# anitasyang/Laplace-GNN

Measured on AMD Instinct MI355X. Metric: la.fit() samples/sec (GCN, KFAC), higher is better.
Workload: dtype f32; 1 GPU; arxiv-shaped 2-layer GCN, hessian_structure=kron (BASELINE configs[2]); num_nodes=169343, nnz=2501719, features=128, hidden=256, classes=40, n_train=90941, batch_size=10000, batches=10, parallelism=dp1 ((batch, class) units, contiguous balanced runs)

## Files before the change

### laplace-gnn_amd/csrc/paths_fused.hip

```cpp
#include "gram256.h"
#include "paths.h"

namespace lgnn {
namespace {

constexpr int kYStride = 272;
constexpr int kPlaneDwords = 512;
constexpr int kGroupDwords = 3 * kPlaneDwords;
constexpr int kYGroups = kYRows / 4;
__device__ __forceinline__ int piece_swap(int q) { return (q ^ (q >> 2)) & 1; }
__device__ __forceinline__ int piece_col(int c) { return 8 * (c >> 2) + 4 * (((c >> 1) & 1) ^ piece_swap(c >> 2)) + 2 * (c & 1); }

struct alignas(16) FusedShared {
  union {
    uint32_t pc[2][kYGroups][3][kPlaneDwords];
    float y[2][kYRows][kYStride];
  };
  int ready[4], done[4];
};
static_assert(sizeof(FusedShared) <= 160 * 1024, "the CU's LDS");

__device__ __forceinline__ int lds_min4(const int* c) {
  int4 v;
  asm volatile("ds_read_b128 %0, %1\n\ts_waitcnt lgkmcnt(0)" : "=v"(v) : "v"(uint32_t(reinterpret_cast<uintptr_t>(c))) : "memory");
  return __builtin_amdgcn_readfirstlane(min(min(v.x, v.y), min(v.z, v.w)));
}
__device__ __forceinline__ void lds_publish(int* c, int value, int lane) {
  if (lane == 0)
    asm volatile("ds_write_b32 %0, %1\n\ts_waitcnt lgkmcnt(0)" :: "v"(uint32_t(reinterpret_cast<uintptr_t>(c))), "v"(value) : "memory");
}

using i32x4 = int __attribute__((ext_vector_type(4)));
__device__ __forceinline__ i32x4 make_rsrc(const void* p, uint64_t bytes) {
  const uint64_t u = reinterpret_cast<uint64_t>(p);
  return i32x4{int(uint32_t(u)), int(uint32_t(u >> 32) & 0xffffu), int(uint32_t(bytes > 0xffffffffull ? 0xffffffffull : bytes)),
               0x00020000};
}
template <bool LIST>
struct NodeRanges {
  i32x4 prs, lrs;
  uint32_t r;
  int64_t base, cnt;
  uint32_t n0;
  __device__ __forceinline__ void init(const int32_t* __restrict__ pptr, const int32_t* __restrict__ list, int64_t n0_, int64_t N,
                                       int64_t nn, int64_t cnt_) {
    prs = make_rsrc(pptr, uint64_t(N + 1) * 4);
    lrs = make_rsrc(LIST ? list : pptr, uint64_t(LIST ? nn : 0) * 4);
    n0 = uint32_t(n0_); cnt = cnt_;
    fill(0);
  }
  __device__ __forceinline__ void fill(int64_t b) {
    base = b;
    const uint32_t ii = uint32_t(b) + (threadIdx.x & 31u);
    const bool in = int64_t(ii) < cnt;
    const uint32_t k = blockIdx.x + ii * gridDim.x;
    uint32_t node = k;
    if constexpr (LIST)
      asm volatile("buffer_load_dword %0, %1, %2, 0 offen\n\ts_waitcnt vmcnt(0)" : "=&v"(node) : "v"(in ? k * 4u : 0xfffffff0u), "s"(lrs) : "memory");
    const uint32_t off = in ? (n0 + node) * 4u + ((threadIdx.x >> 3) & 4u) : 0xfffffff0u;
    asm volatile("buffer_load_dword %0, %1, %2, 0 offen\n\ts_waitcnt vmcnt(0)" : "=&v"(r) : "v"(off), "s"(prs) : "memory");
  }
  __device__ __forceinline__ void get(int64_t i, int32_t& p0, int32_t& p1) {
    if (i - base >= 32) fill(i);
    const int l = int(i - base);
    p0 = __builtin_amdgcn_readlane(int(r), l); p1 = __builtin_amdgcn_readlane(int(r), l + 32);
  }
};

template <int OFF>
__device__ __forceinline__ void bload4(f32x4& d, uint32_t voff, const i32x4& rsrc) {
  asm volatile("buffer_load_dwordx4 %0, %1, %2, 0 offen offset:%3" : "=v"(d) : "v"(voff), "s"(rsrc), "n"(OFF) : "memory");
}
__device__ __forceinline__ void bload1(uint32_t& d, uint32_t voff, const i32x4& rsrc) {
  asm volatile("buffer_load_dword %0, %1, %2, 0 offen" : "=v"(d) : "v"(voff), "s"(rsrc) : "memory");
}
using bf16x8 = __attribute__((ext_vector_type(8))) __bf16;
using u32x4v = __attribute__((ext_vector_type(4))) uint32_t;
using u32x2v = __attribute__((ext_vector_type(2))) uint32_t;

__device__ __forceinline__ uint32_t pk_bf16(float lo, float hi) {
  using bf16x2 = __attribute__((ext_vector_type(2))) __bf16;
  const bf16x2 v = {static_cast<__bf16>(lo), static_cast<__bf16>(hi)};
  return __builtin_bit_cast(uint32_t, v);
}
__device__ __forceinline__ void split_pair(float ya, float yb, uint32_t& q0, uint32_t& q1, uint32_t& q2) {
  q0 = pk_bf16(ya, yb);
  asm("" : "+v"(q0));
  const float r1a = ya - __uint_as_float(q0 << 16), r1b = yb - __uint_as_float(q0 & 0xffff0000u);
  q1 = pk_bf16(r1a, r1b);
  asm("" : "+v"(q1));
  q2 = pk_bf16(r1a - __uint_as_float(q1 << 16), r1b - __uint_as_float(q1 & 0xffff0000u));
}

struct PTables {
  i32x4 coef, b, g, mask, pm, pv, pw;
};

struct PMeta { uint32_t oc, ob, om, w; };
__device__ __forceinline__ void meta_issue(const PTables& tb, int32_t p0, int32_t p1, int lane, PMeta& t) {
  const uint32_t q = uint32_t(max(min(p0 + lane, p1 - 1), 0)) * 4u;
  bload1(t.oc, q, tb.pm);
  bload1(t.om, q, tb.pv);
  bload1(t.w, q, tb.pw);
}
template <int YOUNGER>
__device__ __forceinline__ void meta_finish(int32_t p0, int32_t p1, int lane, uint32_t row_bytes, uint32_t mask_bytes, PMeta& t) {
  asm volatile("s_waitcnt vmcnt(%3)" : "+v"(t.oc), "+v"(t.om), "+v"(t.w) : "n"(YOUNGER) : "memory");
  const bool in = p0 + lane < p1;
  const uint32_t m = in ? t.oc : 0u, v = in ? t.om : 0u;
  t.oc = m * uint32_t(kCoefRow * 4); t.ob = m * row_bytes; t.om = v * mask_bytes;
  t.w = in ? t.w : 0u;
}

struct PLane {
  int kq;
  uint32_t oc, ob, om;
  int mshift;
};

struct POps {
  f32x4 ca[3];
  f32x4 b4, g4;
  uint32_t mw;
  float w;
};

template <bool NOBG> constexpr int kStepLoads = NOBG ? 2 : 6;
template <bool NOBG>
__device__ __forceinline__ void p_load(const PTables& tb, const PMeta& mt, int s, const PLane& pl, POps& o) {
  const int src = 4 * s + pl.kq;
  const uint32_t oc = uint32_t(__shfl(int(mt.oc), src)) + pl.oc;
  const uint32_t om = uint32_t(__shfl(int(mt.om), src)) + pl.om;
  o.w = __uint_as_float(uint32_t(__shfl(int(mt.w), src)));
  bload4<0>(o.ca[0], oc, tb.coef);
  if constexpr (!NOBG) {
    const uint32_t ob = uint32_t(__shfl(int(mt.ob), src)) + pl.ob;
    bload4<kCoefStride * 4>(o.ca[1], oc, tb.coef);
    bload4<2 * kCoefStride * 4>(o.ca[2], oc, tb.coef);
    bload4<0>(o.b4, ob, tb.b);
    bload4<0>(o.g4, ob, tb.g);
  }
  bload1(o.mw, om, tb.mask);
}
template <bool NOBG, int YOUNGER>
__device__ __forceinline__ void p_wait(POps& o) {
  if constexpr (NOBG)
    asm volatile("s_waitcnt vmcnt(%2)" : "+v"(o.ca[0]), "+v"(o.mw) : "n"(YOUNGER) : "memory");
  else
    asm volatile("s_waitcnt vmcnt(%6)" : "+v"(o.ca[0]), "+v"(o.ca[1]), "+v"(o.ca[2]), "+v"(o.b4), "+v"(o.g4), "+v"(o.mw)
                 : "n"(YOUNGER) : "memory");
}

struct PCur { float a1[3], a2[3], bb[4], gg[4]; };
struct PAlpha { u32x4v a[3], m[4]; };
constexpr uint32_t kHiHalves = 0x07060302u;
template <bool NOBG, bool HI, bool SB>
__device__ __forceinline__ void p_xform(const POps& o, const PLane& pl, PCur& c, PAlpha& al, bool bg) {
#pragma unroll
  for (int t = 0; t < 3; ++t) {
    const int tt = HI ? 3 : t;
    if (HI && t > 0) {
      if constexpr (!SB) al.a[t][0] = 0u;
      al.a[t][1] = 0u; al.a[t][2] = 0u;
      continue;
    }
    float av = o.w * o.ca[0][tt];
    asm("" : "+v"(av));
    const uint32_t h0 = __float_as_uint(av) & 0xffff0000u;
    const float r1 = av - __uint_as_float(h0);
    const float r2 = r1 - __uint_as_float(__float_as_uint(r1) & 0xffff0000u);
    if constexpr (!SB) {
      al.a[t][0] = __builtin_amdgcn_perm(__float_as_uint(r1), __float_as_uint(av), kHiHalves);
      al.a[t][1] = __float_as_uint(r2) >> 16;
    } else {
      al.a[t][1] |= h0;
      al.a[t][2] = __builtin_amdgcn_perm(__float_as_uint(r2), __float_as_uint(r1), kHiHalves);
    }
  }
  const int bits = int(o.mw >> pl.mshift);
#pragma unroll
  for (int ct = 0; ct < 4; ++ct) {
    const int on = __builtin_amdgcn_sbfe(bits, ct, 1);
    if constexpr (!SB) {
      al.m[ct][0] = uint32_t(on) & 0x3f803f80u;
      al.m[ct][1] = uint32_t(on) & 0x00003f80u;
    } else {
      al.m[ct][1] |= uint32_t(on) & 0x3f800000u;
      al.m[ct][2] = uint32_t(on) & 0x3f803f80u;
    }
  }
  if constexpr (!NOBG) {
    if (bg) {
#pragma unroll
      for (int t = 0; t < 3; ++t) {
        const int tt = HI ? 3 : t;
        c.a1[t] = (HI && t > 0) ? 0.f : o.w * o.ca[1][tt];
        c.a2[t] = (HI && t > 0) ? 0.f : o.w * o.ca[2][tt];
      }
#pragma unroll
      for (int ct = 0; ct < 4; ++ct) {
        const int on = __builtin_amdgcn_sbfe(bits, ct, 1);
        c.bb[ct] = __uint_as_float(uint32_t(on) & __float_as_uint(o.b4[ct]));
        c.gg[ct] = __uint_as_float(uint32_t(on) & __float_as_uint(o.g4[ct]));
      }
    }
  }
}
template <bool NOBG>
__device__ __forceinline__ void p_keep(const PCur& c) {
  if constexpr (!NOBG) {
    asm volatile("" :: "v"(c.a1[0]), "v"(c.a1[1]), "v"(c.a1[2]), "v"(c.a2[0]), "v"(c.a2[1]), "v"(c.a2[2]));
    asm volatile("" :: "v"(c.bb[0]), "v"(c.bb[1]), "v"(c.bb[2]), "v"(c.bb[3]), "v"(c.gg[0]), "v"(c.gg[1]), "v"(c.gg[2]), "v"(c.gg[3]));
  }
}
__device__ __forceinline__ f32x4 mfma_bf16(u32x4v a, u32x4v b, f32x4 c) {
  return __builtin_amdgcn_mfma_f32_16x16x32_bf16(__builtin_bit_cast(bf16x8, a), __builtin_bit_cast(bf16x8, b), c, 0, 0, 0);
}
__device__ __forceinline__ void p_mfma(const PCur& c, f32x4 (&y2)[3][4]) {
#pragma unroll
  for (int t = 0; t < 3; ++t)
#pragma unroll
    for (int ct = 0; ct < 4; ++ct) y2[t][ct] = __builtin_amdgcn_mfma_f32_16x16x4f32(c.a1[t], c.bb[ct], y2[t][ct], 0, 0, 0);
#pragma unroll
  for (int t = 0; t < 3; ++t)
#pragma unroll
    for (int ct = 0; ct < 4; ++ct) y2[t][ct] = __builtin_amdgcn_mfma_f32_16x16x4f32(c.a2[t], c.gg[ct], y2[t][ct], 0, 0, 0);
}
__device__ __forceinline__ void p_mfma_first(const PCur& c, f32x4 (&y2)[3][4]) {
  const f32x4 zero = {0.f, 0.f, 0.f, 0.f};
#pragma unroll
  for (int t = 0; t < 3; ++t)
#pragma unroll
    for (int ct = 0; ct < 4; ++ct) y2[t][ct] = __builtin_amdgcn_mfma_f32_16x16x4f32(c.a1[t], c.bb[ct], zero, 0, 0, 0);
#pragma unroll
  for (int t = 0; t < 3; ++t)
#pragma unroll
    for (int ct = 0; ct < 4; ++ct) y2[t][ct] = __builtin_amdgcn_mfma_f32_16x16x4f32(c.a2[t], c.gg[ct], y2[t][ct], 0, 0, 0);
}
template <bool FIRST>
__device__ __forceinline__ void p_mfma_alpha(const PAlpha& al, f32x4 (&t1)[3][4]) {
  const f32x4 zero = {0.f, 0.f, 0.f, 0.f};
#pragma unroll
  for (int t = 0; t < 3; ++t)
#pragma unroll
    for (int ct = 0; ct < 4; ++ct) t1[t][ct] = mfma_bf16(al.a[t], al.m[ct], FIRST ? zero : t1[t][ct]);
}

template <bool LIST>
struct ChunkGen {
  int64_t gi;
  int32_t gp, gend;
  int32_t pa0, pa1;
  NodeRanges<LIST> nr;
  __device__ __forceinline__ void init(const int32_t* __restrict__ pptr, const int32_t* __restrict__ list, int64_t n0, int64_t N,
                                       int64_t nn, int64_t cnt) {
    nr.init(pptr, list, n0, N, nn, cnt);
    gi = 0;
    nr.get(0, gp, gend);
    nr.get(1, pa0, pa1);
  }
  __device__ __forceinline__ void next(int64_t cnt, int32_t& q0, int32_t& q1, bool& last) {
    q0 = gp; q1 = min(gp + 64, gend);
    last = q1 >= gend;
    if (last) {
      ++gi;
      gp = pa0; gend = pa1;
      nr.get(gi + 1, pa0, pa1);
    } else {
      gp = q1;
    }
  }
};

template <bool NOBG, bool HI>
__device__ __forceinline__ void pair_body(const PTables& tb, const PMeta& mx, int sx, const PLane& pl, POps& A, POps& B, PCur& cA,
                                          PCur& cB, PAlpha& al, f32x4 (&t1)[3][4], f32x4 (&y2)[3][4], bool first, bool half) {
  constexpr int NL = kStepLoads<NOBG>;
  p_wait<NOBG, NL>(A);
  p_xform<NOBG, HI, false>(A, pl, cA, al, true);
  p_keep<NOBG>(cB);
  p_load<NOBG>(tb, mx, sx, pl, A);
  if constexpr (!NOBG) {
    if (first) p_mfma_first(cA, y2);
    else p_mfma(cA, y2);
  }
  p_wait<NOBG, NL>(B);
  p_xform<NOBG, HI, true>(B, pl, cB, al, !half);
  p_keep<NOBG>(cA);
  p_load<NOBG>(tb, mx, sx + 1, pl, B);
  if (first) p_mfma_alpha<true>(al, t1);
  else p_mfma_alpha<false>(al, t1);
  if constexpr (!NOBG)
    if (!half) p_mfma(cB, y2);
}
template <bool LIST, bool NOBG, bool HI>
__device__ __forceinline__ void product_role(const YArgs& a, const int32_t* __restrict__ pptr, const int32_t* __restrict__ list,
                                             FusedShared& sh, int64_t nn, int64_t cnt, int cg) {
  const int lane = threadIdx.x & 63;
  const int H = a.H;
  const bool path_wave = 64 * cg < H;
  if (!path_wave) return;
  PLane pl;
  const int li = lane & 15;
  pl.kq = lane >> 4;
  const int col = 64 * cg + 4 * li;
  const bool col_ok = col < H;
  pl.oc = 16u * uint32_t(li);
  pl.ob = col_ok ? 4u * uint32_t(col) : 0u;
  pl.om = col_ok ? 4u * uint32_t(col >> 5) : 0x7ffffff0u;
  pl.mshift = col & 31;
  const uint32_t row_bytes = uint32_t(H) * 4u, mask_bytes = uint32_t(a.mask_words) * 4u;
  PTables tb;
  tb.coef = make_rsrc(a.coef, uint64_t(a.n_coef) * kCoefRow * 4);
  tb.b = make_rsrc(a.bg, uint64_t(a.M) * row_bytes);
  tb.g = make_rsrc(a.bg + a.M * int64_t(H), uint64_t(a.M) * row_bytes);
  tb.mask = make_rsrc(a.mask, uint64_t(a.N) * mask_bytes);
  tb.pm = make_rsrc(a.pm, uint64_t(a.cap) * 4);
  tb.pv = make_rsrc(a.pv, uint64_t(a.cap) * 4);
  tb.pw = make_rsrc(a.pw, uint64_t(a.cap) * 4);
  const uint32_t w1_row_bytes = uint32_t(a.w1_ld) * 4u;
  const i32x4 w1rs = make_rsrc(a.W1 + int64_t(a.c0) * a.w1_ld, uint64_t(a.R - 1) * w1_row_bytes + row_bytes);
  constexpr int NL = kStepLoads<NOBG>;
  ChunkGen<LIST> gen;
  gen.init(pptr, list, a.n0, a.N, nn, cnt);
  int32_t q0c, q1c, q0n, q1n;
  bool lastc, lastn;
  gen.next(cnt, q0c, q1c, lastc);
  gen.next(cnt, q0n, q1n, lastn);
  PMeta mc, mn;
  meta_issue(tb, q0c, q1c, lane, mc);
  meta_issue(tb, q0n, q1n, lane, mn);
  meta_finish<0>(q0c, q1c, lane, row_bytes, mask_bytes, mc);
  meta_finish<0>(q0n, q1n, lane, row_bytes, mask_bytes, mn);
  POps A, B;
  p_load<NOBG>(tb, mc, 0, pl, A);
  p_load<NOBG>(tb, mc, 1, pl, B);
  f32x4 t1[3][4], y2[3][4];
#pragma unroll
  for (int t = 0; t < 3; ++t)
#pragma unroll
    for (int ct = 0; ct < 4; ++ct) { t1[t][ct] = f32x4{0.f, 0.f, 0.f, 0.f}; y2[t][ct] = f32x4{0.f, 0.f, 0.f, 0.f}; }
  PCur cA = {}, cB = {};
  PAlpha al;
#pragma unroll
  for (int t = 0; t < 3; ++t) al.a[t] = u32x4v{0u, 0u, 0u, 0u};
#pragma unroll
  for (int ct = 0; ct < 4; ++ct) al.m[ct] = u32x4v{0u, 0u, 0u, 0u};
  bool node_has = false;
  bool firstc = true;
  for (int64_t i = 0; i < cnt;) {
    int32_t q0f, q1f;
    bool lastf;
    gen.next(cnt, q0f, q1f, lastf);
    PMeta mf2;
    meta_issue(tb, q0f, q1f, lane, mf2);
    const int kch = q1c - q0c, np = max((kch + 7) >> 3, 1);
    node_has = node_has || kch > 0;
#pragma clang loop unroll(disable)
    for (int j = 0; j < np; ++j) {
      const bool more = j + 1 < np;
      PMeta mx;
      mx.oc = more ? mc.oc : mn.oc; mx.ob = more ? mc.ob : mn.ob; mx.om = more ? mc.om : mn.om; mx.w = more ? mc.w : mn.w;
      const int sx = more ? 2 * (j + 1) : 0;
      const bool first = firstc && j == 0, half = !more && 4 * (2 * j + 1) >= kch;
      pair_body<NOBG, HI>(tb, mx, sx, pl, A, B, cA, cB, al, t1, y2, first, half);
    }
    if (lastc) {
      int wl = lane;
      asm volatile("" : "+v"(wl));
      const int wkq = wl >> 4, wcol = 64 * cg + 4 * (wl & 15);
      const bool wcol_ok = wcol < H;
      const uint32_t w1_off = wcol_ok ? uint32_t(4 * wkq) * w1_row_bytes + 4u * uint32_t(wcol) : 0x7ff00000u;
      const int pc_lo = 8 * (wcol >> 2) + 4 * piece_swap(wcol >> 2), pc_hi = pc_lo ^ 4;
      f32x4 w1[3][4];
#pragma unroll
      for (int t = 0; t < 3; ++t)
#pragma unroll
        for (int r = 0; r < 4; ++r) bload4<0>(w1[t][r], w1_off + uint32_t(16 * t + r) * w1_row_bytes, w1rs);
      if (i >= 2)
        while (lds_min4(sh.done) < int(i) - 1) __builtin_amdgcn_s_sleep(2);
#pragma unroll
      for (int t = 0; t < 3; ++t)
        asm volatile("s_waitcnt vmcnt(0)" : "+v"(w1[t][0]), "+v"(w1[t][1]), "+v"(w1[t][2]), "+v"(w1[t][3]) :: "memory");
      asm volatile("s_nop 11" ::: "memory");
      __builtin_amdgcn_sched_barrier(0);
      if (node_has && wcol_ok) {
        if (a.gram_f32) {
          float (*ytile)[kYStride] = sh.y[i & 1];
#pragma unroll
          for (int t = 0; t < 3; ++t)
#pragma unroll
            for (int r = 0; r < 4; ++r) {
              f32x4 o;
#pragma unroll
              for (int ct = 0; ct < 4; ++ct) o[ct] = w1[t][r][ct] * t1[t][ct][r] + y2[t][ct][r];
              *reinterpret_cast<f32x4*>(&ytile[16 * t + 4 * wkq + r][wcol]) = o;
            }
        } else {
          uint32_t* __restrict__ grp = &sh.pc[i & 1][wkq][0][0];
#pragma unroll
          for (int t = 0; t < 3; ++t) {
            u32x4v pz[3][2];
#pragma unroll
            for (int ct = 0; ct < 4; ++ct)
#pragma unroll
              for (int rp = 0; rp < 2; ++rp) {
                const float ya = w1[t][2 * rp][ct] * t1[t][ct][2 * rp] + y2[t][ct][2 * rp];
                const float yb = w1[t][2 * rp + 1][ct] * t1[t][ct][2 * rp + 1] + y2[t][ct][2 * rp + 1];
                uint32_t q0, q1, q2;
                split_pair(ya, yb, q0, q1, q2);
                pz[0][ct >> 1][2 * (ct & 1) + rp] = q0;
                pz[1][ct >> 1][2 * (ct & 1) + rp] = q1;
                pz[2][ct >> 1][2 * (ct & 1) + rp] = q2;
              }
            uint32_t* __restrict__ g = grp + 4 * t * kGroupDwords;
            *reinterpret_cast<u32x4v*>(g + pc_lo) = pz[2][0];
            *reinterpret_cast<u32x4v*>(g + pc_hi) = pz[2][1];
            *reinterpret_cast<u32x4v*>(g + kPlaneDwords + pc_lo) = pz[0][0];
            *reinterpret_cast<u32x4v*>(g + kPlaneDwords + pc_hi) = pz[0][1];
            *reinterpret_cast<u32x4v*>(g + 2 * kPlaneDwords + pc_lo) = pz[1][0];
            *reinterpret_cast<u32x4v*>(g + 2 * kPlaneDwords + pc_hi) = pz[1][1];
          }
        }
      }
      ++i;
      lds_publish(&sh.ready[cg], int(i), lane);
#pragma unroll
      for (int t = 0; t < 3; ++t) {
        asm volatile("" : "=v"(t1[t][0]), "=v"(t1[t][1]), "=v"(t1[t][2]), "=v"(t1[t][3]));
        if constexpr (!NOBG) asm volatile("" : "=v"(y2[t][0]), "=v"(y2[t][1]), "=v"(y2[t][2]), "=v"(y2[t][3]));
      }
      node_has = false;
    }
    meta_finish<2 * NL>(q0f, q1f, lane, row_bytes, mask_bytes, mf2);
    firstc = lastc;
    q0c = q0n; q1c = q1n; lastc = lastn; mc = mn;
    q0n = q0f; q1n = q1f; lastn = lastf; mn = mf2;
  }
  asm volatile("s_waitcnt vmcnt(0)" ::: "memory");
}

template <int W>
__device__ __forceinline__ void gram16_load(const float* __restrict__ p, float (&x)[8][2]) {
#pragma unroll
  for (int b = 0; b < 8; ++b) {
    x[b][0] = tiles256_uses<W>(b) ? p[b * 32] : 0.f;
    x[b][1] = tiles256_uses<W>(b) ? p[b * 32 + 16] : 0.f;
  }
}
template <int W>
__device__ __forceinline__ void gram16_mfma(const float (&x)[8][2], f32x4 (&acc)[9][2][2]) {
#pragma unroll
  for (int s = 0; s < 9; ++s)
#pragma unroll
    for (int hi = 0; hi < 2; ++hi)
#pragma unroll
      for (int hj = 0; hj < 2; ++hj) {
        if (Tiles256<W>::si[s] == Tiles256<W>::sj[s] && hi > hj) continue;
        acc[s][hi][hj] = __builtin_amdgcn_mfma_f32_16x16x4f32(x[Tiles256<W>::si[s]][hi], x[Tiles256<W>::sj[s]][hj],
                                                              acc[s][hi][hj], 0, 0, 0);
      }
}
template <int W, bool LIST>
__device__ __forceinline__ void gram_role(const YArgs& a, const int32_t* __restrict__ pptr, const int32_t* __restrict__ list,
                                          FusedShared& sh, int64_t nn, int64_t cnt, float* __restrict__ scratch) {
  const int lane = threadIdx.x & 63;
  f32x4 acc[9][2][2];
#pragma unroll
  for (int s = 0; s < 9; ++s)
#pragma unroll
    for (int q = 0; q < 4; ++q) acc[s][q >> 1][q & 1] = f32x4{0.f, 0.f, 0.f, 0.f};
  const int nk = (a.R + 3) >> 2;
  NodeRanges<LIST> nr;
  nr.init(pptr, list, a.n0, a.N, nn, cnt);
  int32_t p0, p1;
  nr.get(0, p0, p1);
  for (int64_t i = 0; i < cnt; ++i) {
    int32_t q0, q1;
    nr.get(i + 1, q0, q1);
    while (lds_min4(sh.ready) < int(i) + 1) __builtin_amdgcn_s_sleep(2);
    if (p1 > p0) {
      const float* __restrict__ base = &sh.y[i & 1][0][0] + (lane >> 4) * kYStride + (lane & 15);
      float xa[8][2], xb[8][2];
      gram16_load<W>(base, xa);
      for (int kk = 0; kk < nk; kk += 2) {
        if (kk + 1 < nk) gram16_load<W>(base + (kk + 1) * 4 * kYStride, xb);
        __builtin_amdgcn_sched_barrier(0);
        gram16_mfma<W>(xa, acc);
        __builtin_amdgcn_sched_barrier(0);
        if (kk + 1 < nk) {
          if (kk + 2 < nk) gram16_load<W>(base + (kk + 2) * 4 * kYStride, xa);
          __builtin_amdgcn_sched_barrier(0);
          gram16_mfma<W>(xb, acc);
          __builtin_amdgcn_sched_barrier(0);
        }
      }
    }
    lds_publish(&sh.done[W], int(i) + 1, lane);
    p0 = q0; p1 = q1;
  }
  const int64_t D = a.H;
  const int li = lane & 15, lq = lane >> 4;
#pragma unroll
  for (int s = 0; s < 9; ++s)
#pragma unroll
    for (int hi = 0; hi < 2; ++hi)
#pragma unroll
      for (int hj = 0; hj < 2; ++hj) {
        if (Tiles256<W>::si[s] == Tiles256<W>::sj[s] && hi > hj) continue;
        const int64_t jj = Tiles256<W>::sj[s] * 32 + 16 * hj + li;
#pragma unroll
        for (int r = 0; r < 4; ++r) {
          const int64_t ii = Tiles256<W>::si[s] * 32 + 16 * hi + 4 * lq + r;
          if (ii < D && jj < D) atomicAdd(&scratch[ii * D + jj], acc[s][hi][hj][r]);
        }
      }
}

struct PieceBlk { u32x4v t; u32x2v y1; };

template <int W> struct GramOrder;
template <> struct GramOrder<0> { static constexpr int o[9] = {0, 3, 4, 7, 8, 1, 2, 5, 6}; };
template <> struct GramOrder<1> { static constexpr int o[9] = {7, 8, 3, 4, 5, 6, 0, 1, 2}; };
template <> struct GramOrder<2> { static constexpr int o[9] = {7, 8, 3, 4, 5, 6, 0, 1, 2}; };
template <> struct GramOrder<3> { static constexpr int o[9] = {0, 7, 3, 5, 1, 8, 4, 6, 2}; };
template <int W> __device__ __forceinline__ constexpr int gram_last_use(int b) {
  int last = -1;
  for (int p = 0; p < 9; ++p)
    if (Tiles256<W>::si[GramOrder<W>::o[p]] == b || Tiles256<W>::sj[GramOrder<W>::o[p]] == b) last = p;
  return last;
}
template <int W> __device__ __forceinline__ constexpr int gram_first_use(int b) {
  for (int p = 0; p < 9; ++p)
    if (Tiles256<W>::si[GramOrder<W>::o[p]] == b || Tiles256<W>::sj[GramOrder<W>::o[p]] == b) return p;
  return -1;
}

__device__ __forceinline__ void piece_load(const uint32_t* __restrict__ tile, int off, int b, PieceBlk (&x)[8][2]) {
  const uint32_t* __restrict__ pe = tile + off;
  const uint32_t* __restrict__ po = tile + (off ^ 4) + 32;
  const u32x2v e2 = *reinterpret_cast<const u32x2v*>(pe + b * 64), e0 = *reinterpret_cast<const u32x2v*>(pe + kPlaneDwords + b * 64);
  const u32x2v o2 = *reinterpret_cast<const u32x2v*>(po + b * 64), o0 = *reinterpret_cast<const u32x2v*>(po + kPlaneDwords + b * 64);
  x[b][0].t = u32x4v{e2[0], e2[1], e0[0], e0[1]};
  x[b][0].y1 = *reinterpret_cast<const u32x2v*>(pe + 2 * kPlaneDwords + b * 64);
  x[b][1].t = u32x4v{o2[0], o2[1], o0[0], o0[1]};
  x[b][1].y1 = *reinterpret_cast<const u32x2v*>(po + 2 * kPlaneDwords + b * 64);
}
__device__ __forceinline__ u32x4v piece_u(const PieceBlk& p) { return u32x4v{p.t[2], p.t[3], p.y1[0], p.y1[1]}; }
__device__ __forceinline__ u32x4v piece_t(const PieceBlk& p) { return p.t; }
template <int W>
__device__ __forceinline__ void piece_chunk16(PieceBlk (&x)[8][2], f32x4 (&acc)[9][2][2], const uint32_t* __restrict__ tile, int off) {
#pragma unroll
  for (int p = 0; p < 9; ++p) {
    const int s = GramOrder<W>::o[p], si = Tiles256<W>::si[s], sj = Tiles256<W>::sj[s];
#pragma unroll
    for (int b = 0; b < 8; ++b)
      if (gram_first_use<W>(b) == p)
#pragma unroll
        for (int h = 0; h < 2; ++h) asm volatile("" : "+v"(x[b][h].t), "+v"(x[b][h].y1));
    const u32x4v ua[2] = {piece_u(x[si][0]), piece_u(x[si][1])}, ta[2] = {piece_t(x[si][0]), piece_t(x[si][1])};
    const u32x4v ub[2] = {piece_u(x[sj][0]), piece_u(x[sj][1])}, tb[2] = {piece_t(x[sj][0]), piece_t(x[sj][1])};
#pragma unroll
    for (int f = 0; f < 3; ++f)
#pragma unroll
      for (int hi = 0; hi < 2; ++hi)
#pragma unroll
        for (int hj = 0; hj < 2; ++hj) {
          if (si == sj && hi > hj) continue;
          acc[s][hi][hj] = mfma_bf16(f == 1 ? ta[hi] : ua[hi], f == 2 ? tb[hj] : ub[hj], acc[s][hi][hj]);
        }
    __builtin_amdgcn_sched_barrier(0);
#pragma unroll
    for (int b = 0; b < 8; ++b)
      if (gram_last_use<W>(b) == p) piece_load(tile, off, b, x);
  }
}
template <int W>
__device__ __forceinline__ void piece_chunk8(const PieceBlk (&x)[8][2], f32x4 (&acc)[9][2][2], bool low) {
#pragma unroll
  for (int p = 0; p < 9; ++p) {
    const int s = GramOrder<W>::o[p], si = Tiles256<W>::si[s], sj = Tiles256<W>::sj[s];
    u32x4v a1[2], a2[2];
#pragma unroll
    for (int hi = 0; hi < 2; ++hi) {
      const u32x4v u = piece_u(x[si][hi]), t = piece_t(x[si][hi]);
#pragma unroll
      for (int j = 0; j < 4; ++j) { a1[hi][j] = low ? u[j] : t[j]; a2[hi][j] = low ? u[j] : 0u; }
    }
    const u32x4v ub[2] = {piece_u(x[sj][0]), piece_u(x[sj][1])}, tb[2] = {piece_t(x[sj][0]), piece_t(x[sj][1])};
#pragma unroll
    for (int f = 0; f < 2; ++f)
#pragma unroll
      for (int hi = 0; hi < 2; ++hi)
#pragma unroll
        for (int hj = 0; hj < 2; ++hj) {
          if (si == sj && hi > hj) continue;
          acc[s][hi][hj] = mfma_bf16(f == 0 ? a1[hi] : a2[hi], f == 0 ? ub[hj] : tb[hj], acc[s][hi][hj]);
        }
    __builtin_amdgcn_sched_barrier(0);
  }
}
template <int W, bool LIST>
__device__ __forceinline__ void gram_split16_role(const YArgs& a, const int32_t* __restrict__ pptr, const int32_t* __restrict__ list,
                                                  FusedShared& sh, int64_t nn, int64_t cnt, float* __restrict__ scratch) {
  const int lane = threadIdx.x & 63;
  f32x4 acc[9][2][2];
#pragma unroll
  for (int s = 0; s < 9; ++s)
#pragma unroll
    for (int q = 0; q < 4; ++q) acc[s][q >> 1][q & 1] = f32x4{0.f, 0.f, 0.f, 0.f};
  const int n8 = (a.R + 7) >> 3, n16 = n8 >> 1;
  const bool odd = n8 & 1;
  const int gq = lane >> 4;
  const int start = (n16 > 0 ? gq : gq & 1) * kGroupDwords + piece_col(lane & 15);
  const int to_odd = (4 - 2 * (gq >> 1)) * kGroupDwords;
  NodeRanges<LIST> nr;
  nr.init(pptr, list, a.n0, a.N, nn, cnt);
  int32_t p0, p1;
  nr.get(0, p0, p1);
  for (int64_t i = 0; i < cnt; ++i) {
    int32_t q0, q1;
    nr.get(i + 1, q0, q1);
    while (lds_min4(sh.ready) < int(i) + 1) __builtin_amdgcn_s_sleep(2);
    if (p1 > p0) {
      const uint32_t* __restrict__ tile = &sh.pc[i & 1][0][0][0];
      int off = start;
      PieceBlk x[8][2];
#pragma unroll
      for (int b = 0; b < 8; ++b)
        if (tiles256_uses<W>(b)) piece_load(tile, off, b, x);
      __builtin_amdgcn_sched_barrier(0);
      for (int cc = 0; cc < n16; ++cc) {
        off += cc + 1 < n16 ? 4 * kGroupDwords : odd ? to_odd : 0;
        piece_chunk16<W>(x, acc, tile, off);
      }
      if (odd) piece_chunk8<W>(x, acc, gq < 2);
    }
    lds_publish(&sh.done[W], int(i) + 1, lane);
    p0 = q0; p1 = q1;
  }
  const int64_t D = a.H;
  const int fl = int(__builtin_amdgcn_mbcnt_hi(~0u, __builtin_amdgcn_mbcnt_lo(~0u, 0u)));
  const int li = fl & 15, lq = (fl >> 4) & 3;
#pragma unroll
  for (int s = 0; s < 9; ++s)
#pragma unroll
    for (int hi = 0; hi < 2; ++hi)
#pragma unroll
      for (int hj = 0; hj < 2; ++hj) {
        if (Tiles256<W>::si[s] == Tiles256<W>::sj[s] && hi > hj) continue;
        const int64_t jj = Tiles256<W>::sj[s] * 32 + 16 * hj + li;
#pragma unroll
        for (int r = 0; r < 4; ++r) {
          const int64_t ii = Tiles256<W>::si[s] * 32 + 16 * hi + 4 * lq + r;
          if (ii < D && jj < D && (Tiles256<W>::si[s] != Tiles256<W>::sj[s] || ii <= jj)) atomicAdd(&scratch[ii * D + jj], acc[s][hi][hj][r]);
        }
      }
}

template <bool LIST>
__global__ __launch_bounds__(512, 2) void paths_fused_kernel(YArgs a, const int32_t* __restrict__ pptr,
                                                             const int32_t* __restrict__ list, float* __restrict__ scratch) {
  __shared__ FusedShared sh;
  if (int64_t(pptr[a.N]) > a.cap) return;
  for (int q = threadIdx.x; q < int(sizeof(sh.pc) / 16); q += 512) reinterpret_cast<u32x4v*>(&sh.pc[0][0][0][0])[q] = u32x4v{0u, 0u, 0u, 0u};
  if (threadIdx.x < 4) {
    sh.ready[threadIdx.x] = 64 * int(threadIdx.x) < a.H ? 0 : INT32_MAX;
    sh.done[threadIdx.x] = 0;
  }
  __syncthreads();
  const int hw = __builtin_amdgcn_readfirstlane(int(threadIdx.x >> 6));
  const int64_t stride = gridDim.x;
  const int64_t nn = LIST ? int64_t(__builtin_amdgcn_readfirstlane(*a.n_list)) : a.n1 - a.n0;
  const int64_t cnt = nn > int64_t(blockIdx.x) ? (nn - blockIdx.x + stride - 1) / stride : 0;
  switch (hw) {
    case 4: if (a.gram_f32) gram_role<0, LIST>(a, pptr, list, sh, nn, cnt, scratch); else gram_split16_role<0, LIST>(a, pptr, list, sh, nn, cnt, scratch); break;
    case 5: if (a.gram_f32) gram_role<1, LIST>(a, pptr, list, sh, nn, cnt, scratch); else gram_split16_role<1, LIST>(a, pptr, list, sh, nn, cnt, scratch); break;
    case 6: if (a.gram_f32) gram_role<2, LIST>(a, pptr, list, sh, nn, cnt, scratch); else gram_split16_role<2, LIST>(a, pptr, list, sh, nn, cnt, scratch); break;
    case 7: if (a.gram_f32) gram_role<3, LIST>(a, pptr, list, sh, nn, cnt, scratch); else gram_split16_role<3, LIST>(a, pptr, list, sh, nn, cnt, scratch); break;
    default:
      if (a.c0 != a.cb) {
        if (a.no_bg) product_role<LIST, true, true>(a, pptr, list, sh, nn, cnt, hw);
        else product_role<LIST, false, true>(a, pptr, list, sh, nn, cnt, hw);
      } else {
        if (a.no_bg) product_role<LIST, true, false>(a, pptr, list, sh, nn, cnt, hw);
        else product_role<LIST, false, false>(a, pptr, list, sh, nn, cnt, hw);
      }
      break;
  }
}

constexpr int64_t kFusedWorkgroups = 256;

}

int launch_paths_fused(lgnn_ctx* h, YArgs y, int64_t cb, int64_t ce, float* scratch, hipStream_t s) {
  LGNN_REQUIRE(y.N < (int64_t(1) << 31), "too many nodes for one launch");
  const dim3 grid{unsigned(std::min<int64_t>(y.n1 - y.n0, kFusedWorkgroups))};
  const char* e = getenv("LGNN_GRAM_F32");
  y.Y = nullptr; y.gram_f32 = e && atoi(e) != 0 ? 1 : 0;
  for (int64_t c0 = cb; c0 < ce; c0 += kYRows) {
    y.c0 = int(c0); y.R = int(std::min<int64_t>(kYRows, ce - c0));
    if (h->timing) LGNN_CALL(record_event(h, s));
    if (y.list) hipLaunchKernelGGL(paths_fused_kernel<true>, grid, dim3(512), 0, s, y, y.pptr, y.list, scratch);
    else hipLaunchKernelGGL(paths_fused_kernel<false>, grid, dim3(512), 0, s, y, y.pptr, y.list, scratch);
    LGNN_HIP_CHECK(hipGetLastError());
    if (h->timing) { LGNN_CALL(record_event(h, s)); h->ev_planes += y.R; }
  }
  return 0;
}

}
```

Before: 2.528 million samples/s.

## Stage first W1 tiles in LDS and shrink tile buffers for short row chunks

Replaces the fixed union shared-memory struct with a runtime-sized LDS layout. When the f32 gram path is used or the chunk has few rows, the first two 16-row tiles of W1 are preloaded into LDS at kernel start, so the product waves read them with ds_read instead of buffer loads in every node epilogue; only the third tile still comes from global memory. The split16 tile buffer is shortened for short chunks to make room for this. It also inserts s_nop padding before several buffer loads, adds LDS pressure and more template instantiations, and under the non-HI product path with the default split16 layout, W1 is staged only when the chunk has at most 40 rows.

```diff
diff --git a/laplace-gnn_amd/csrc/paths_fused.hip b/laplace-gnn_amd/csrc/paths_fused.hip
--- a/laplace-gnn_amd/csrc/paths_fused.hip
+++ b/laplace-gnn_amd/csrc/paths_fused.hip
@@ -11,14 +11,32 @@
 __device__ __forceinline__ int piece_swap(int q) { return (q ^ (q >> 2)) & 1; }
 __device__ __forceinline__ int piece_col(int c) { return 8 * (c >> 2) + 4 * (((c >> 1) & 1) ^ piece_swap(c >> 2)) + 2 * (c & 1); }
 
-struct alignas(16) FusedShared {
-  union {
-    uint32_t pc[2][kYGroups][3][kPlaneDwords];
-    float y[2][kYRows][kYStride];
-  };
-  int ready[4], done[4];
+constexpr int kW1Cols = 256;
+constexpr int kW1Tiles = 2;
+constexpr int kShortGroups = 10, kShortRows = 4 * kShortGroups;
+constexpr int fused_tile_dwords(bool f32, int R) {
+  return f32 ? kYRows * kYStride : kGroupDwords * (R <= kShortRows ? kShortGroups : kYGroups);
+}
+constexpr int fused_w1_tiles(bool f32, int R) { return f32 || R <= kShortRows ? kW1Tiles : 0; }
+constexpr int fused_lds_bytes(bool f32, int R) {
+  return 4 * (2 * fused_tile_dwords(f32, R) + fused_w1_tiles(f32, R) * 16 * kW1Cols) + 32;
+}
+constexpr int kFusedLdsBytes = fused_lds_bytes(false, kShortRows);
+static_assert(kFusedLdsBytes == 155680 && kFusedLdsBytes <= 160 * 1024, "the CU's LDS");
+static_assert(fused_lds_bytes(false, kYRows) <= kFusedLdsBytes && fused_lds_bytes(true, kYRows) <= kFusedLdsBytes &&
+              fused_lds_bytes(true, 1) <= kFusedLdsBytes && fused_lds_bytes(false, 1) <= kFusedLdsBytes, "every layout fits");
+struct FusedShared {
+  uint32_t* base;
+  int tile_dwords;
+  int nw;
+  __device__ __forceinline__ void init(uint32_t* lds, bool f32, int R) {
+    base = lds; tile_dwords = fused_tile_dwords(f32, R); nw = fused_w1_tiles(f32, R);
+  }
+  __device__ __forceinline__ uint32_t* tile(int64_t i) const { return base + (int(i) & 1) * tile_dwords; }
+  __device__ __forceinline__ float* w1() const { return reinterpret_cast<float*>(base + 2 * tile_dwords); }
+  __device__ __forceinline__ int* ready() const { return reinterpret_cast<int*>(base + 2 * tile_dwords + nw * 16 * kW1Cols); }
+  __device__ __forceinline__ int* done() const { return ready() + 4; }
 };
-static_assert(sizeof(FusedShared) <= 160 * 1024, "the CU's LDS");
 
 __device__ __forceinline__ int lds_min4(const int* c) {
   int4 v;
@@ -28,6 +46,17 @@
 __device__ __forceinline__ void lds_publish(int* c, int value, int lane) {
   if (lane == 0)
     asm volatile("ds_write_b32 %0, %1\n\ts_waitcnt lgkmcnt(0)" :: "v"(uint32_t(reinterpret_cast<uintptr_t>(c))), "v"(value) : "memory");
+}
+
+template <int T>
+__device__ __forceinline__ void w1_lds_read(f32x4 (&w)[4], uint32_t addr) {
+  asm volatile("ds_read_b128 %0, %1 offset:%2" : "=v"(w[0]) : "v"(addr), "n"((16 * T + 0) * kW1Cols * 4) : "memory");
+  asm volatile("ds_read_b128 %0, %1 offset:%2" : "=v"(w[1]) : "v"(addr), "n"((16 * T + 1) * kW1Cols * 4) : "memory");
+  asm volatile("ds_read_b128 %0, %1 offset:%2" : "=v"(w[2]) : "v"(addr), "n"((16 * T + 2) * kW1Cols * 4) : "memory");
+  asm volatile("ds_read_b128 %0, %1 offset:%2" : "=v"(w[3]) : "v"(addr), "n"((16 * T + 3) * kW1Cols * 4) : "memory");
+}
+__device__ __forceinline__ void w1_lds_wait(f32x4 (&w)[4]) {
+  asm volatile("s_waitcnt lgkmcnt(0)" : "+v"(w[0]), "+v"(w[1]), "+v"(w[2]), "+v"(w[3]) :: "memory");
 }
 
 using i32x4 = int __attribute__((ext_vector_type(4)));
@@ -56,9 +85,9 @@
     const uint32_t k = blockIdx.x + ii * gridDim.x;
     uint32_t node = k;
     if constexpr (LIST)
-      asm volatile("buffer_load_dword %0, %1, %2, 0 offen\n\ts_waitcnt vmcnt(0)" : "=&v"(node) : "v"(in ? k * 4u : 0xfffffff0u), "s"(lrs) : "memory");
+      asm volatile("s_nop 4\n\tbuffer_load_dword %0, %1, %2, 0 offen\n\ts_waitcnt vmcnt(0)" : "=&v"(node) : "v"(in ? k * 4u : 0xfffffff0u), "s"(lrs) : "memory");
     const uint32_t off = in ? (n0 + node) * 4u + ((threadIdx.x >> 3) & 4u) : 0xfffffff0u;
-    asm volatile("buffer_load_dword %0, %1, %2, 0 offen\n\ts_waitcnt vmcnt(0)" : "=&v"(r) : "v"(off), "s"(prs) : "memory");
+    asm volatile("s_nop 4\n\tbuffer_load_dword %0, %1, %2, 0 offen\n\ts_waitcnt vmcnt(0)" : "=&v"(r) : "v"(off), "s"(prs) : "memory");
   }
   __device__ __forceinline__ void get(int64_t i, int32_t& p0, int32_t& p1) {
     if (i - base >= 32) fill(i);
@@ -67,12 +96,17 @@
   }
 };
 
-template <int OFF>
+template <int OFF, bool PAD = false>
 __device__ __forceinline__ void bload4(f32x4& d, uint32_t voff, const i32x4& rsrc) {
-  asm volatile("buffer_load_dwordx4 %0, %1, %2, 0 offen offset:%3" : "=v"(d) : "v"(voff), "s"(rsrc), "n"(OFF) : "memory");
-}
+  if constexpr (PAD)
+    asm volatile("s_nop 4\n\tbuffer_load_dwordx4 %0, %1, %2, 0 offen offset:%3" : "=v"(d) : "v"(voff), "s"(rsrc), "n"(OFF) : "memory");
+  else
+    asm volatile("buffer_load_dwordx4 %0, %1, %2, 0 offen offset:%3" : "=v"(d) : "v"(voff), "s"(rsrc), "n"(OFF) : "memory");
+}
+template <bool PAD = false>
 __device__ __forceinline__ void bload1(uint32_t& d, uint32_t voff, const i32x4& rsrc) {
-  asm volatile("buffer_load_dword %0, %1, %2, 0 offen" : "=v"(d) : "v"(voff), "s"(rsrc) : "memory");
+  if constexpr (PAD) asm volatile("s_nop 4\n\tbuffer_load_dword %0, %1, %2, 0 offen" : "=v"(d) : "v"(voff), "s"(rsrc) : "memory");
+  else asm volatile("buffer_load_dword %0, %1, %2, 0 offen" : "=v"(d) : "v"(voff), "s"(rsrc) : "memory");
 }
 using bf16x8 = __attribute__((ext_vector_type(8))) __bf16;
 using u32x4v = __attribute__((ext_vector_type(4))) uint32_t;
@@ -99,9 +133,9 @@
 struct PMeta { uint32_t oc, ob, om, w; };
 __device__ __forceinline__ void meta_issue(const PTables& tb, int32_t p0, int32_t p1, int lane, PMeta& t) {
   const uint32_t q = uint32_t(max(min(p0 + lane, p1 - 1), 0)) * 4u;
-  bload1(t.oc, q, tb.pm);
-  bload1(t.om, q, tb.pv);
-  bload1(t.w, q, tb.pw);
+  bload1<true>(t.oc, q, tb.pm);
+  bload1<true>(t.om, q, tb.pv);
+  bload1<true>(t.w, q, tb.pw);
 }
 template <int YOUNGER>
 __device__ __forceinline__ void meta_finish(int32_t p0, int32_t p1, int lane, uint32_t row_bytes, uint32_t mask_bytes, PMeta& t) {
@@ -293,9 +327,9 @@
   if constexpr (!NOBG)
     if (!half) p_mfma(cB, y2);
 }
-template <bool LIST, bool NOBG, bool HI>
+template <bool LIST, bool NOBG, bool HI, bool W1L>
 __device__ __forceinline__ void product_role(const YArgs& a, const int32_t* __restrict__ pptr, const int32_t* __restrict__ list,
-                                             FusedShared& sh, int64_t nn, int64_t cnt, int cg) {
+                                             const FusedShared& sh, int64_t nn, int64_t cnt, int cg) {
   const int lane = threadIdx.x & 63;
   const int H = a.H;
   const bool path_wave = 64 * cg < H;
@@ -372,59 +406,80 @@
       const bool wcol_ok = wcol < H;
       const uint32_t w1_off = wcol_ok ? uint32_t(4 * wkq) * w1_row_bytes + 4u * uint32_t(wcol) : 0x7ff00000u;
       const int pc_lo = 8 * (wcol >> 2) + 4 * piece_swap(wcol >> 2), pc_hi = pc_lo ^ 4;
+      constexpr int nw = W1L ? kW1Tiles : 0;
       f32x4 w1[3][4];
 #pragma unroll
-      for (int t = 0; t < 3; ++t)
-#pragma unroll
-        for (int r = 0; r < 4; ++r) bload4<0>(w1[t][r], w1_off + uint32_t(16 * t + r) * w1_row_bytes, w1rs);
+      for (int t = nw; t < 3; ++t)
+#pragma unroll
+        for (int r = 0; r < 4; ++r) bload4<0, true>(w1[t][r], w1_off + uint32_t(16 * t + r) * w1_row_bytes, w1rs);
+      const uint32_t w1_lds = uint32_t(reinterpret_cast<uintptr_t>(sh.w1())) + uint32_t(4 * wkq * kW1Cols * 4 + 4 * wcol);
+      if constexpr (nw > 0) w1_lds_read<0>(w1[0], w1_lds);
       if (i >= 2)
-        while (lds_min4(sh.done) < int(i) - 1) __builtin_amdgcn_s_sleep(2);
-#pragma unroll
-      for (int t = 0; t < 3; ++t)
-        asm volatile("s_waitcnt vmcnt(0)" : "+v"(w1[t][0]), "+v"(w1[t][1]), "+v"(w1[t][2]), "+v"(w1[t][3]) :: "memory");
+        while (lds_min4(sh.done()) < int(i) - 1) __builtin_amdgcn_s_sleep(2);
+      if constexpr (nw > 0) w1_lds_wait(w1[0]);
+      if constexpr (nw == 0) {
+#pragma unroll
+        for (int t = 0; t < 3; ++t)
+          asm volatile("s_waitcnt vmcnt(0)" : "+v"(w1[t][0]), "+v"(w1[t][1]), "+v"(w1[t][2]), "+v"(w1[t][3]) :: "memory");
+      }
       asm volatile("s_nop 11" ::: "memory");
       __builtin_amdgcn_sched_barrier(0);
-      if (node_has && wcol_ok) {
-        if (a.gram_f32) {
-          float (*ytile)[kYStride] = sh.y[i & 1];
-#pragma unroll
-          for (int t = 0; t < 3; ++t)
-#pragma unroll
-            for (int r = 0; r < 4; ++r) {
-              f32x4 o;
-#pragma unroll
-              for (int ct = 0; ct < 4; ++ct) o[ct] = w1[t][r][ct] * t1[t][ct][r] + y2[t][ct][r];
-              *reinterpret_cast<f32x4*>(&ytile[16 * t + 4 * wkq + r][wcol]) = o;
-            }
-        } else {
-          uint32_t* __restrict__ grp = &sh.pc[i & 1][wkq][0][0];
-#pragma unroll
-          for (int t = 0; t < 3; ++t) {
-            u32x4v pz[3][2];
-#pragma unroll
-            for (int ct = 0; ct < 4; ++ct)
-#pragma unroll
-              for (int rp = 0; rp < 2; ++rp) {
-                const float ya = w1[t][2 * rp][ct] * t1[t][ct][2 * rp] + y2[t][ct][2 * rp];
-                const float yb = w1[t][2 * rp + 1][ct] * t1[t][ct][2 * rp + 1] + y2[t][ct][2 * rp + 1];
-                uint32_t q0, q1, q2;
-                split_pair(ya, yb, q0, q1, q2);
-                pz[0][ct >> 1][2 * (ct & 1) + rp] = q0;
-                pz[1][ct >> 1][2 * (ct & 1) + rp] = q1;
-                pz[2][ct >> 1][2 * (ct & 1) + rp] = q2;
-              }
-            uint32_t* __restrict__ g = grp + 4 * t * kGroupDwords;
-            *reinterpret_cast<u32x4v*>(g + pc_lo) = pz[2][0];
-            *reinterpret_cast<u32x4v*>(g + pc_hi) = pz[2][1];
-            *reinterpret_cast<u32x4v*>(g + kPlaneDwords + pc_lo) = pz[0][0];
-            *reinterpret_cast<u32x4v*>(g + kPlaneDwords + pc_hi) = pz[0][1];
-            *reinterpret_cast<u32x4v*>(g + 2 * kPlaneDwords + pc_lo) = pz[1][0];
-            *reinterpret_cast<u32x4v*>(g + 2 * kPlaneDwords + pc_hi) = pz[1][1];
+      const bool wr = node_has && wcol_ok;
+      uint32_t* __restrict__ tile = sh.tile(i);
+      auto f32_tile = [&](auto tc) __attribute__((always_inline)) {
+        constexpr int t = decltype(tc)::value;
+        if constexpr (t + 1 < nw) w1_lds_read<t + 1>(w1[t + 1], w1_lds);
+        float (*ytile)[kYStride] = reinterpret_cast<float (*)[kYStride]>(tile);
+#pragma unroll
+        for (int r = 0; r < 4; ++r) {
+          f32x4 o;
+#pragma unroll
+          for (int ct = 0; ct < 4; ++ct) o[ct] = w1[t][r][ct] * t1[t][ct][r] + y2[t][ct][r];
+          *reinterpret_cast<f32x4*>(&ytile[16 * t + 4 * wkq + r][wcol]) = o;
+        }
+        if constexpr (t + 1 < nw) w1_lds_wait(w1[t + 1]);
+      };
+      auto piece_tile = [&](auto tc) __attribute__((always_inline)) {
+        constexpr int t = decltype(tc)::value;
+        if constexpr (t + 1 < nw) w1_lds_read<t + 1>(w1[t + 1], w1_lds);
+        u32x4v pz[3][2];
+#pragma unroll
+        for (int ct = 0; ct < 4; ++ct)
+#pragma unroll
+          for (int rp = 0; rp < 2; ++rp) {
+            const float ya = w1[t][2 * rp][ct] * t1[t][ct][2 * rp] + y2[t][ct][2 * rp];
+            const float yb = w1[t][2 * rp + 1][ct] * t1[t][ct][2 * rp + 1] + y2[t][ct][2 * rp + 1];
+            uint32_t q0, q1, q2;
+            split_pair(ya, yb, q0, q1, q2);
+            pz[0][ct >> 1][2 * (ct & 1) + rp] = q0;
+            pz[1][ct >> 1][2 * (ct & 1) + rp] = q1;
+            pz[2][ct >> 1][2 * (ct & 1) + rp] = q2;
           }
+        if constexpr (t + 1 < nw) w1_lds_wait(w1[t + 1]);
+        if (t < 2 || sh.tile_dwords != kGroupDwords * kShortGroups || wkq < kShortGroups - 8) {
+          uint32_t* __restrict__ g = tile + (4 * t + wkq) * kGroupDwords;
+          *reinterpret_cast<u32x4v*>(g + pc_lo) = pz[2][0];
+          *reinterpret_cast<u32x4v*>(g + pc_hi) = pz[2][1];
+          *reinterpret_cast<u32x4v*>(g + kPlaneDwords + pc_lo) = pz[0][0];
+          *reinterpret_cast<u32x4v*>(g + kPlaneDwords + pc_hi) = pz[0][1];
+          *reinterpret_cast<u32x4v*>(g + 2 * kPlaneDwords + pc_lo) = pz[1][0];
+          *reinterpret_cast<u32x4v*>(g + 2 * kPlaneDwords + pc_hi) = pz[1][1];
         }
+      };
+      using T0 = std::integral_constant<int, 0>; using T1 = std::integral_constant<int, 1>; using T2 = std::integral_constant<int, 2>;
+      if (wr) {
+        if (a.gram_f32) { f32_tile(T0{}); f32_tile(T1{}); if constexpr (nw == 0) f32_tile(T2{}); }
+        else { piece_tile(T0{}); piece_tile(T1{}); if constexpr (nw == 0) piece_tile(T2{}); }
+      }
+      if constexpr (nw > 0) {
+        asm volatile("s_waitcnt vmcnt(0)" : "+v"(w1[2][0]), "+v"(w1[2][1]), "+v"(w1[2][2]), "+v"(w1[2][3]) :: "memory");
+        if (wr) {
+          if (a.gram_f32) f32_tile(T2{});
+          else piece_tile(T2{});
+        }
       }
       ++i;
-      lds_publish(&sh.ready[cg], int(i), lane);
+      lds_publish(sh.ready() + cg, int(i), lane);
 #pragma unroll
       for (int t = 0; t < 3; ++t) {
         asm volatile("" : "=v"(t1[t][0]), "=v"(t1[t][1]), "=v"(t1[t][2]), "=v"(t1[t][3]));
@@ -463,7 +518,7 @@
 }
 template <int W, bool LIST>
 __device__ __forceinline__ void gram_role(const YArgs& a, const int32_t* __restrict__ pptr, const int32_t* __restrict__ list,
-                                          FusedShared& sh, int64_t nn, int64_t cnt, float* __restrict__ scratch) {
+                                          const FusedShared& sh, int64_t nn, int64_t cnt, float* __restrict__ scratch) {
   const int lane = threadIdx.x & 63;
   f32x4 acc[9][2][2];
 #pragma unroll
@@ -478,9 +533,9 @@
   for (int64_t i = 0; i < cnt; ++i) {
     int32_t q0, q1;
     nr.get(i + 1, q0, q1);
-    while (lds_min4(sh.ready) < int(i) + 1) __builtin_amdgcn_s_sleep(2);
+    while (lds_min4(sh.ready()) < int(i) + 1) __builtin_amdgcn_s_sleep(2);
     if (p1 > p0) {
-      const float* __restrict__ base = &sh.y[i & 1][0][0] + (lane >> 4) * kYStride + (lane & 15);
+      const float* __restrict__ base = reinterpret_cast<const float*>(sh.tile(i)) + (lane >> 4) * kYStride + (lane & 15);
       float xa[8][2], xb[8][2];
       gram16_load<W>(base, xa);
       for (int kk = 0; kk < nk; kk += 2) {
@@ -496,7 +551,7 @@
         }
       }
     }
-    lds_publish(&sh.done[W], int(i) + 1, lane);
+    lds_publish(sh.done() + W, int(i) + 1, lane);
     p0 = q0; p1 = q1;
   }
   const int64_t D = a.H;
@@ -602,7 +657,7 @@
 }
 template <int W, bool LIST>
 __device__ __forceinline__ void gram_split16_role(const YArgs& a, const int32_t* __restrict__ pptr, const int32_t* __restrict__ list,
-                                                  FusedShared& sh, int64_t nn, int64_t cnt, float* __restrict__ scratch) {
+                                                  const FusedShared& sh, int64_t nn, int64_t cnt, float* __restrict__ scratch) {
   const int lane = threadIdx.x & 63;
   f32x4 acc[9][2][2];
 #pragma unroll
@@ -621,9 +676,9 @@
   for (int64_t i = 0; i < cnt; ++i) {
     int32_t q0, q1;
     nr.get(i + 1, q0, q1);
-    while (lds_min4(sh.ready) < int(i) + 1) __builtin_amdgcn_s_sleep(2);
+    while (lds_min4(sh.ready()) < int(i) + 1) __builtin_amdgcn_s_sleep(2);
     if (p1 > p0) {
-      const uint32_t* __restrict__ tile = &sh.pc[i & 1][0][0][0];
+      const uint32_t* __restrict__ tile = sh.tile(i);
       int off = start;
       PieceBlk x[8][2];
 #pragma unroll
@@ -636,7 +691,7 @@
       }
       if (odd) piece_chunk8<W>(x, acc, gq < 2);
     }
-    lds_publish(&sh.done[W], int(i) + 1, lane);
+    lds_publish(sh.done() + W, int(i) + 1, lane);
     p0 = q0; p1 = q1;
   }
   const int64_t D = a.H;
@@ -661,12 +716,20 @@
 template <bool LIST>
 __global__ __launch_bounds__(512, 2) void paths_fused_kernel(YArgs a, const int32_t* __restrict__ pptr,
                                                              const int32_t* __restrict__ list, float* __restrict__ scratch) {
-  __shared__ FusedShared sh;
+  __shared__ alignas(16) uint32_t lds[kFusedLdsBytes / 4];
   if (int64_t(pptr[a.N]) > a.cap) return;
-  for (int q = threadIdx.x; q < int(sizeof(sh.pc) / 16); q += 512) reinterpret_cast<u32x4v*>(&sh.pc[0][0][0][0])[q] = u32x4v{0u, 0u, 0u, 0u};
+  FusedShared sh;
+  sh.init(lds, a.gram_f32 != 0, a.R);
+  for (int q = threadIdx.x; q < 2 * sh.tile_dwords / 4; q += 512) reinterpret_cast<u32x4v*>(sh.base)[q] = u32x4v{0u, 0u, 0u, 0u};
+  for (int q = threadIdx.x; q < sh.nw * 16 * (kW1Cols / 4); q += 512) {
+    const int row = q / (kW1Cols / 4), c4 = 4 * (q % (kW1Cols / 4));
+    f32x4 v = {0.f, 0.f, 0.f, 0.f};
+    if (row < a.R && c4 < a.H) v = *reinterpret_cast<const f32x4*>(a.W1 + (int64_t(a.c0) + row) * a.w1_ld + c4);
+    reinterpret_cast<f32x4*>(sh.w1())[q] = v;
+  }
   if (threadIdx.x < 4) {
-    sh.ready[threadIdx.x] = 64 * int(threadIdx.x) < a.H ? 0 : INT32_MAX;
-    sh.done[threadIdx.x] = 0;
+    sh.ready()[threadIdx.x] = 64 * int(threadIdx.x) < a.H ? 0 : INT32_MAX;
+    sh.done()[threadIdx.x] = 0;
   }
   __syncthreads();
   const int hw = __builtin_amdgcn_readfirstlane(int(threadIdx.x >> 6));
@@ -680,11 +743,14 @@
     case 7: if (a.gram_f32) gram_role<3, LIST>(a, pptr, list, sh, nn, cnt, scratch); else gram_split16_role<3, LIST>(a, pptr, list, sh, nn, cnt, scratch); break;
     default:
       if (a.c0 != a.cb) {
-        if (a.no_bg) product_role<LIST, true, true>(a, pptr, list, sh, nn, cnt, hw);
-        else product_role<LIST, false, true>(a, pptr, list, sh, nn, cnt, hw);
+        if (a.no_bg) product_role<LIST, true, true, true>(a, pptr, list, sh, nn, cnt, hw);
+        else product_role<LIST, false, true, true>(a, pptr, list, sh, nn, cnt, hw);
+      } else if (sh.nw > 0) {
+        if (a.no_bg) product_role<LIST, true, false, true>(a, pptr, list, sh, nn, cnt, hw);
+        else product_role<LIST, false, false, true>(a, pptr, list, sh, nn, cnt, hw);
       } else {
-        if (a.no_bg) product_role<LIST, true, false>(a, pptr, list, sh, nn, cnt, hw);
-        else product_role<LIST, false, false>(a, pptr, list, sh, nn, cnt, hw);
+        if (a.no_bg) product_role<LIST, true, false, false>(a, pptr, list, sh, nn, cnt, hw);
+        else product_role<LIST, false, false, false>(a, pptr, list, sh, nn, cnt, hw);
       }
       break;
   }
```

Result: slower. 2.484 million samples/s (-1.7%).
